# tylerrleee/mcmc-gpu

Measured on AMD Instinct MI355X. Metric: chain-steps/sec on 256x256 grid x 1024 chains; accept-rate parity, higher is better.
Workload: dtype f64; 1 GPU; largeScaleChain 256x256 grid, 1024 chains/GPU, fp64, Philox spectral (Matern 0.9125) proposals, blocks 50-80, sigma_mc 5 (BASELINE configs[1]); chains_total=1024, mh_steps_per_bench_step=2048

## Files before the change

mcmc_gpu_amd/csrc/chain_strip_kernel.hip:

```cpp
#include "gsm_internal.h"
#include "device_util.h"
#include "proposal_device.h"
#include "strip_step.h"
#include <math.h>
#include <stdlib.h>
#include <algorithm>
#include <type_traits>

namespace gsm {

using namespace dev;
using strip::kST;
using strip::kSW;
using strip::kNR;

constexpr int kSUPW = 32 / kSW;
constexpr int kSMAXT = 16 / kSW;

static int strip_tile_len(const BlockTable& B) { return (B.max_bh + 2) * (B.max_bw + 2); }
static int strip_main_len(const FusedArgs& a) { return std::max(a.P.lds_main, strip_tile_len(a.T.B)); }
constexpr int kStripAux = 16 + 32 + 16 + kMathTabDoubles + 4 * kT1S + kMask1D;
size_t fused_strip_lds_doubles(const FusedArgs& a) { return (size_t)strip_main_len(a) + kStripAux; }

bool strip_table_ok(const StaticFields& S, const BlockTable& B, int lds_main, int tiles1_max, int tiles2_max) {
  static int on = -1;
  if (on < 0) { const char* v = getenv("GSM_STRIP"); on = v ? atoi(v) : 1; }
  const size_t lds = ((size_t)std::max(lds_main, strip_tile_len(B)) + kStripAux) * sizeof(double);
  return on && S.sA != nullptr && (uint64_t)S.H * S.W * 48u <= (4ull << 20) && B.n_sizes <= 64 && strip::table_ok(B.max_bh, B.max_bw) &&
         B.max_bh <= kT1S && B.max_bw <= kT1S && (B.masks == nullptr || B.mask1d != nullptr) && lds <= 80 * 1024 && 2 * tiles1_max <= kSW * kSUPW && tiles2_max <= kSW * kSMAXT;
}

using step::crec_t;
using step::load_c;

template <typename TS, bool FAST_DIV, bool NOISE>
__global__ __launch_bounds__(kST, 4) void chain_strip_kernel(const FusedArgs fa) {
  typedef step::cptr_t<FusedArgs> cargs_t;
  auto kargs = [] { return step::kargs<FusedArgs>(); };
  extern __shared__ double lds[];
  double* __restrict__ red = lds + fa.work_len;
  double* __restrict__ red2 = red + 16;
  double* __restrict__ carry = red2 + 32;
  double* __restrict__ mtab = red2 + 32 + 16;
// ... 108 lines not shown
        relaunder();
        nugget_pass<kST, NOISE>(ptid, pa, q, pg, seed, pa.step0 + s, nz, lds, [bw](int y, int x) { return (y + 1) * (bw + 2) + x + 1; }, mtab);
      }
    }
    relaunder();
    const step::Window Gw = step::clip_window(gH, gW, s_row, s_col, s_bh, s_bw);
    strip::Window G;
    {
      const cargs_t K = kargs();
      G = strip::make_window(gH, gW, s_row, s_col, s_bh, s_bw, K->T.S.tr0, K->T.S.tr1, K->T.S.tc0, K->T.S.tc1);
    }
    const strip::Cfg cfg = strip::config(G.wh, G.ww);
    const strip::Lane L = strip::lane_setup(ptid & 63, wave, cfg, G, gH, gW);
    const rsrc_t r_bed = make_rsrc(p_bed, n_cells * (uint32_t)sizeof(TS));
    const rsrc_t r_en = make_rsrc(p_en, n_cells * (uint32_t)sizeof(TS));
    const rsrc_t r_st = make_rsrc(p_st, 3u * n_cells * 16u);
    uint32_t upd_bits;
    double acc_old;
    bool guard;
    {
      double vb[kNR + 2], ve[kNR];
      double2 a2[strip::kNA];
      if (G.interior) strip::load_state<TS, true>(L, cfg.n, gW, r_bed, r_en, r_st, vb, ve, a2);
      else strip::load_state<TS, false>(L, cfg.n, gW, r_bed, r_en, r_st, vb, ve, a2);
      asm volatile("s_waitcnt lgkmcnt(0)\n\ts_barrier" ::: "memory");
      const int ts = s_bw + 2;
      auto field = [&](int jj, bool) { return lds[L.tidx + jj * ts]; };
      if (G.interior) strip::phase_a<TS, true>(L, cfg.n, gW, s_bw, r_st, field, lds, vb, ve, a2, upd_bits, acc_old, guard);
      else strip::phase_a<TS, false>(L, cfg.n, gW, s_bw, r_st, field, lds, vb, ve, a2, upd_bits, acc_old, guard);
    }
    asm volatile("s_waitcnt lgkmcnt(0)\n\ts_barrier" ::: "memory");
    double en[kNR], vn[kNR];
    {
      double acc_new;
      const cargs_t K = kargs();
      const step::StepConsts SC{K->T.S.res, K->T.S.rcp_res, K->T.S.two_res, K->T.S.rcp_two_res};
      if (G.interior) strip::phase_d<TS, FAST_DIV, true>(L, cfg.n, gW, s_bw, r_st, n_cells * 16u, SC, lds, en, acc_new);
      else strip::phase_d<TS, FAST_DIV, false>(L, cfg.n, gW, s_bw, r_st, n_cells * 16u, SC, lds, en, acc_new);
      double delta = acc_new - acc_old;
      if (guard) delta = INFINITY;
      const double w_delta = wave64_sum(delta);
      if (lane == 0) red[wave] = w_delta;
    }
    strip::read_candidate(L, cfg.n, s_bw, lds, vn);
    const double s_hi = carry[0], s_lo = carry[1];
    double loss_prev = carry[2];
    asm volatile("s_waitcnt lgkmcnt(0)\n\ts_barrier" ::: "memory");
    const double sd = strip::waves_sum(red, lane);
    double c_hi, c_lo, loss_next;
    const bool acc = step::decide<FAST_DIV>(sd, sd == INFINITY, s_hi, s_lo, two_sigma2, rcp_two_sigma2, loss_prev, rec->u, c_hi, c_lo, loss_next);
    if (acc) {
      if (G.interior) strip::commit<TS, true, false>(L, cfg.n, gW, r_bed, r_en, r_en, vn, en, upd_bits);
      else strip::commit<TS, false, false>(L, cfg.n, gW, r_bed, r_en, r_en, vn, en, upd_bits);
// ... 23 lines not shown
__global__ __launch_bounds__(kST, 4) void step_strip_kernel(const StepArgs a) {
  extern __shared__ double tile[];
  __shared__ double red[16];
  __shared__ int tab[2 * 64];
  const StaticFields& S = a.S;
  const int tid = threadIdx.x;
  const int lane = tid & 63;
  const int wave = __builtin_amdgcn_readfirstlane(tid >> 6);
  const int chain = blockIdx.x;
  const int H = S.H, W = S.W;
  const uint32_t n_cells = (uint32_t)H * (uint32_t)W;
  const size_t plane = (size_t)H * W;
  const rsrc_t r_bed = make_rsrc((const TS*)a.beds + (size_t)chain * plane, n_cells * (uint32_t)sizeof(TS));
  const rsrc_t r_en = make_rsrc((const TS*)a.energy + (size_t)chain * plane, n_cells * (uint32_t)sizeof(TS));
  const rsrc_t r_rs = make_rsrc(a.resampled + (size_t)chain * plane, n_cells * 4u);
  const rsrc_t r_st = make_rsrc(S.sA, 3u * n_cells * 16u);
  const step::StepConsts SC{S.res, S.rcp_res, S.two_res, S.rcp_two_res};

  double s_hi = a.loss_sum[2 * chain], s_lo = a.loss_sum[2 * chain + 1];
  double loss_prev = (s_hi + s_lo) / S.two_sigma2;
  for (int i = tid; i < a.B.n_sizes; i += kST) { tab[2 * i] = a.B.bh[i]; tab[2 * i + 1] = a.B.bw[i]; }
  if (tid < 16) red[tid] = 0.0;
  const int64_t rin0 = (int64_t)chain * a.in_stride;
  step::ReplayRec nxt = step::read_replay(a, rin0);
  __syncthreads();

  for (int s = 0; s < a.n_steps; ++s) {
    const int64_t rin = rin0 + s;
    const int64_t rout = step::record_index(a, chain, s);
    const step::ReplayRec cur = nxt;
    const bool has_next = s + 1 < a.n_steps;
// ... 4 lines not shown
    }
    const int bh = tab[2 * cur.si], bw = tab[2 * cur.si + 1];
    const rsrc_t r_f = make_rsrc(a.fields + rin * a.field_stride, (uint32_t)(bh * bw) * 8u);
    strip::Window G;
    {
      const step::cptr_t<StepArgs> K = step::kargs<StepArgs>();
      G = strip::uniform(strip::make_window(H, W, cur.row, cur.col, bh, bw, K->S.tr0, K->S.tr1, K->S.tc0, K->S.tc1));
    }
    const strip::Cfg cfg = strip::config(G.wh, G.ww);
    const strip::Lane L = strip::lane_setup(lane, wave, cfg, G, H, W);
    uint32_t upd_bits;
    double acc_old;
    bool guard;
    {
      double vb[kNR + 2], ve[kNR];
      double2 a2[strip::kNA];
      auto field = [&](int jj, bool in) { return ld_f64<2>(r_f, in ? (uint32_t)(L.fidx + jj * bw) * 8u : kOOB); };
      if (G.interior) {
        strip::load_state<TS, true>(L, cfg.n, W, r_bed, r_en, r_st, vb, ve, a2);
        strip::phase_a<TS, true>(L, cfg.n, W, bw, r_st, field, tile, vb, ve, a2, upd_bits, acc_old, guard);
      } else {
        strip::load_state<TS, false>(L, cfg.n, W, r_bed, r_en, r_st, vb, ve, a2);
        strip::phase_a<TS, false>(L, cfg.n, W, bw, r_st, field, tile, vb, ve, a2, upd_bits, acc_old, guard);
      }
    }
    asm volatile("s_waitcnt lgkmcnt(0)\n\ts_barrier" ::: "memory");
    double en[kNR], vn[kNR];
    {
      double acc_new;
      if (G.interior) strip::phase_d<TS, FAST_DIV, true>(L, cfg.n, W, bw, r_st, n_cells * 16u, SC, tile, en, acc_new);
      else strip::phase_d<TS, FAST_DIV, false>(L, cfg.n, W, bw, r_st, n_cells * 16u, SC, tile, en, acc_new);
      double delta = acc_new - acc_old;
      if (guard) delta = INFINITY;
      const double w_delta = wave64_sum(delta);
      if (lane == 0) red[wave] = w_delta;
    }
    strip::read_candidate(L, cfg.n, bw, tile, vn);
    asm volatile("s_waitcnt lgkmcnt(0)\n\ts_barrier" ::: "memory");
    const double sd = strip::waves_sum(red, lane);
    double c_hi, c_lo, loss_next;
    const bool acc = step::decide<FAST_DIV>(sd, sd == INFINITY, s_hi, s_lo, S.two_sigma2, S.rcp_two_sigma2, loss_prev, cur.u, c_hi, c_lo, loss_next);
    if (acc) {
      if (G.interior) strip::commit<TS, true, true>(L, cfg.n, W, r_bed, r_en, r_rs, vn, en, upd_bits);
      else strip::commit<TS, false, true>(L, cfg.n, W, r_bed, r_en, r_rs, vn, en, upd_bits);
      two_sum(c_hi, c_lo, s_hi, s_lo);
      loss_prev = loss_next;
// ... 50 lines not shown
```

mcmc_gpu_amd/csrc/device_util.h:

```cpp
#pragma once
#include <hip/hip_runtime.h>
#include <stdint.h>

namespace gsm {
namespace dev {


constexpr int kNT = 1024;
constexpr int kNW = kNT / 64;
constexpr uint32_t kOOB = 0x80000000u;
constexpr uint64_t kNoUpdBits = 0x7FF8DEADBEEF0001ull;

typedef int v2i32 __attribute__((ext_vector_type(2)));
typedef int v4i32 __attribute__((ext_vector_type(4)));
typedef __amdgpu_buffer_rsrc_t rsrc_t;

__device__ __forceinline__ rsrc_t make_rsrc(const void* p, uint32_t bytes) {
  return __builtin_amdgcn_make_buffer_rsrc(const_cast<void*>(p), 0, (int)bytes, 0x00020000);
}
template <int AUX>
__device__ __forceinline__ double ld_f64(rsrc_t r, uint32_t off) {
  return __builtin_bit_cast(double, __builtin_amdgcn_raw_buffer_load_b64(r, (int)off, 0, AUX));
}
template <int AUX>
__device__ __forceinline__ float ld_f32(rsrc_t r, uint32_t off) {
  return __builtin_bit_cast(float, __builtin_amdgcn_raw_buffer_load_b32(r, (int)off, 0, AUX));
// ... 74 lines not shown
```

mcmc_gpu_amd/csrc/gsm_api.hip:

```cpp
#include "gsm_context.h"
#include "math_tables.h"
#include "normal_score.h"
#include <math.h>
#include <string.h>
#include <algorithm>

using namespace gsm;

static thread_local std::string g_create_err;

int gsm::fail(gsm_handle h, int code, const std::string& msg) {
  if (h) h->err = msg; else g_create_err = msg;
  return code;
}

extern "C" const char* gsm_last_error(gsm_handle h) { return h ? h->err.c_str() : g_create_err.c_str(); }

extern "C" int gsm_create(gsm_handle* out, int32_t H, int32_t W, int32_t n_chains, int32_t dtype, int32_t device) {
  if (!out) return fail(nullptr, GSM_E_ARG, "gsm_create: out is NULL");
  *out = nullptr;
  if (H < 1 || W < 1 || n_chains < 1) return fail(nullptr, GSM_E_ARG, "gsm_create: need H,W >= 1 and n_chains >= 1");
  if ((int64_t)H * W > (1LL << 30)) return fail(nullptr, GSM_E_ARG, "gsm_create: grid too large");
  if (dtype != 0 && dtype != 1) return fail(nullptr, GSM_E_UNSUPPORTED, "gsm_create: dtype must be 0 (fp64 state) or 1 (fp32 state)");
  int ndev = 0;
// ... 64 lines not shown
  S.rcp_two_res = 1.0 / S.two_res;
  S.two_sigma2 = 2 * (sigma_mc * sigma_mc);
  S.rcp_two_sigma2 = 1.0 / S.two_sigma2;
  {
    auto divisor_ok = [](double d) {
      uint64_t bits;
      memcpy(&bits, &d, sizeof(bits));
      const bool all_ones = (bits & 0xFFFFFFFFFFFFFull) == 0xFFFFFFFFFFFFFull;
      return !all_ones && d > 1e-100 && d < 1e100;
    };
    S.fast_div = (divisor_ok(S.res) && divisor_ok(S.two_sigma2)) ? 1 : 0;
  }
  HIPCHK(h, h->d_svx.ensure(n));
  HIPCHK(h, h->d_svy.ensure(n));
  HIPCHK(h, h->d_ds.ensure(n));
  HIPCHK(h, h->d_sABC.ensure(3 * n));
  double2 *sA = h->d_sABC.get(), *sB = sA + n, *sC = sA + 2 * n;
  HIPCHK(h, launch_pack_static(S, h->d_svx.get(), h->d_svy.get(), h->d_ds.get(), st));
  HIPCHK(h, launch_pack_flux_static(S, sA, sB, sC, st));
  S.svx = h->d_svx.get(); S.svy = h->d_svy.get(); S.ds = h->d_ds.get();
  S.sA = sA; S.sB = sB; S.sC = sC;
  HIPCHK(h, hipStreamSynchronize(st));
  h->have_static = true;
  return GSM_OK;
}

extern "C" int gsm_set_blocks(gsm_handle h, int32_t n_sizes, const int32_t* bh, const int32_t* bw,
                              const double* edge_masks_packed, const int64_t* mask_offsets, void* stream) {
  GSM_GRID_HANDLE(h);
  if (n_sizes < 1 || !bh || !bw) return fail(h, GSM_E_ARG, "gsm_set_blocks: empty block table");
  if (n_sizes > 64) return fail(h, GSM_E_UNSUPPORTED, "gsm_set_blocks: at most 64 block sizes");
  hipStream_t st = (hipStream_t)stream;
  HIPCHK(h, hipSetDevice(h->device));
  int max_bh = 0, max_bw = 0, cap = 0;
  int64_t mask_total = 0;
  for (int i = 0; i < n_sizes; ++i) {
// ... 350 lines not shown
```

mcmc_gpu_amd/csrc/gsm_internal.h:

```cpp
#pragma once
#include <hip/hip_runtime.h>
#include <stdint.h>
#include <string>
#include <vector>
#include "../../include/gsm.h"

namespace gsm {

constexpr int kMaxDevices = 64;
inline bool attr_needed_on_this_device(bool (&flags)[kMaxDevices], int& dev) {
  dev = 0;
  if (hipGetDevice(&dev) != hipSuccess || dev < 0 || dev >= kMaxDevices) { dev = -1; return true; }
  return !flags[dev];
}
template <auto K0, auto K1, class... Args>
inline hipError_t launch_pair(bool first, int lds_cap, dim3 grid, dim3 block, size_t lds, hipStream_t st, const Args&... args) {
  static bool attr_set[kMaxDevices] = {};
  int attr_dev;
  if (attr_needed_on_this_device(attr_set, attr_dev)) {
    hipError_t e = hipFuncSetAttribute((const void*)K0, hipFuncAttributeMaxDynamicSharedMemorySize, lds_cap);
    if (e == hipSuccess) e = hipFuncSetAttribute((const void*)K1, hipFuncAttributeMaxDynamicSharedMemorySize, lds_cap);
    if (e != hipSuccess) return e;
    if (attr_dev >= 0) attr_set[attr_dev] = true;
  }
// ... 5 lines not shown
struct StaticFields {
  const double* surf;
  const double* velx;
  const double* vely;
  const double* dhdt;
  const double* smb;
  const double* weight;
  const uint8_t* upd;
  const uint8_t* mc;
  const double2* svx;
  const double2* svy;
  const double2* ds;
  const double2* sA;
  const double2* sB;
  const double2* sC;
  int H, W;
  int32_t tr0, tr1, tc0, tc1;
  double res;
  double two_res;
  double rcp_res;
  double rcp_two_res;
  int fast_div;
  double two_sigma2;
  double rcp_two_sigma2;
};

struct BlockTable {
  const int32_t* bh;
  const int32_t* bw;
  const double* masks;
// ... 285 lines not shown
                     double* out, int64_t n, int inverse, hipStream_t st);
hipError_t launch_qt_groups(const double* quantiles, const double* references, int nq, double clip_min, double clip_max, const double* x,
                            double* out, int n_chains, int plane, const int32_t* group, int inverse, hipStream_t st);
hipError_t launch_sgs_commit_map(int H, int W, int n_chains, double* cur, const double* proposed, uint32_t* resampled, const int32_t* win,
                                 const uint8_t* accept, hipStream_t st);
hipError_t launch_sgs_commit(int H, int W, int n_chains, double* cur, double* next, uint32_t* resampled, const int32_t* win,
                             const uint8_t* accept, hipStream_t st);

hipError_t launch_propose_cholesky(const ProposeArgs& a, const CholArgs& c, hipStream_t st);
hipError_t launch_cholesky_upper(double* A, int n, int ld, double jitter, int* d_info, hipStream_t st);
hipError_t launch_cov_assemble(int bh, int bw, double res, const gsm_vario& v, const double* lag_table, double* sigma,
                               int ld, hipStream_t st);
hipError_t launch_step(const StepArgs& a, hipStream_t st);
hipError_t launch_step_flux(const StepArgs& a, hipStream_t st);
bool step_flux_supported(const StepArgs& a);
hipError_t launch_pack_flux_static(const StaticFields& S, double2* sA, double2* sB, double2* sC, hipStream_t st);
hipError_t launch_init_loss(const StaticFields& S, int n_chains, const void* beds, void* energy, int f32_state,
                            double* loss_sum, double* loss0, hipStream_t st);
hipError_t launch_pack_static(const StaticFields& S, double2* svx, double2* svy, double2* ds, hipStream_t st);
hipError_t launch_residual(const StaticFields& S, int n_chains, const double* beds, double* out, hipStream_t st);
hipError_t launch_propose(const ProposeArgs& a, hipStream_t st);
hipError_t launch_propose_scalars(const ProposeArgs& a, hipStream_t st);
hipError_t launch_debug_normals(uint64_t seed, int64_t step, uint32_t stream_id, uint32_t idx0, int n, const double* mathtab, double* out,
                                hipStream_t st);
hipError_t launch_debug_proposal_math(int which, int model, double smoothness, int64_t n, const void* x0, const double* x1, const double* x2,
                                      const double* x3, const double* mathtab, void* out, hipStream_t st);
hipError_t launch_k2_tables(const BlockTable& B, const int32_t* k2_off, double resolution, double* k2tab, hipStream_t st);
hipError_t launch_spectral_from_noise(const ProposeArgs& a, const int32_t* size_idx, const double* rf_scalars, const double* noise_re,
                                      const double* noise_im, const double* nugget_field, hipStream_t st);
hipError_t launch_chain_fused(const FusedArgs& a, hipStream_t st);
hipError_t launch_chain_strip(const FusedArgs& a, hipStream_t st);
// ... 28 lines not shown
```

mcmc_gpu_amd/csrc/step_flux_kernel.hip:

```cpp
#include "gsm_internal.h"
#include "device_util.h"
#include "step_common.h"
#include <math.h>
#include <stdlib.h>
#include <algorithm>

namespace gsm {

using namespace dev;

size_t step_flux_lds_bytes(int tile_cap) { return ((size_t)2 * tile_cap + 4 * kNW + 64) * sizeof(double); }

template <typename TS, int KT, bool FAST_DIV>
__global__ __launch_bounds__(kNT, 4) void step_flux_kernel(const StepArgs a) {
  constexpr bool F32 = sizeof(TS) == 4;
  extern __shared__ double lds[];
  double* __restrict__ qx = lds;
  double* __restrict__ qy = lds + a.tile_cap;
  double* __restrict__ red = lds + 2 * a.tile_cap;
  int* tab = (int*)(red + 4 * kNW);

  const StaticFields& S = a.S;
  const int tid = threadIdx.x;
  const int lane = tid & 63;
// ... 168 lines not shown
         (uint64_t)a.S.H * a.S.W * 16u < 0x80000000ull;
}

hipError_t launch_step_flux(const StepArgs& a, hipStream_t st) {
  if (!step_flux_supported(a)) return hipErrorInvalidValue;
  if (a.f32_state) {
    if (a.tile_cap <= 2 * kNT) return launch_flux_t<float, 2>(a, st);
    if (a.tile_cap <= 4 * kNT) return launch_flux_t<float, 4>(a, st);
    return launch_flux_t<float, 7>(a, st);
  }
  if (a.tile_cap <= 2 * kNT) return launch_flux_t<double, 2>(a, st);
  if (a.tile_cap <= 4 * kNT) return launch_flux_t<double, 4>(a, st);
  return launch_flux_t<double, 7>(a, st);
}

__global__ __launch_bounds__(256) void pack_flux_static_kernel(const StaticFields S, double2* sA, double2* sB, double2* sC) {
  const int n = S.H * S.W;
  for (int g = blockIdx.x * 256 + threadIdx.x; g < n; g += gridDim.x * 256) {
    const double w = S.weight ? S.weight[g] : 1.0;
    sA[g] = make_double2(S.upd[g] ? w : __builtin_bit_cast(double, kNoUpdBits), S.surf[g]);
    sB[g] = make_double2(S.velx[g], S.vely[g]);
    sC[g] = make_double2(S.mc[g] == 1 ? S.dhdt[g] : __builtin_nan(""), S.smb[g]);
  }
}

hipError_t launch_pack_flux_static(const StaticFields& S, double2* sA, double2* sB, double2* sC, hipStream_t st) {
  int grid = (S.H * S.W + 255) / 256;
  if (grid > 2048) grid = 2048;
  hipLaunchKernelGGL(pack_flux_static_kernel, dim3(grid), dim3(256), 0, st, S, sA, sB, sC);
  return hipGetLastError();
}

}
```

mcmc_gpu_amd/csrc/strip_step.h:

```cpp
#pragma once
#include "gsm_internal.h"
#include "device_util.h"
#include "step_common.h"
#include <math.h>

namespace gsm {
namespace strip {

using namespace dev;

constexpr int kST = 512;
constexpr int kSW = kST / 64;
constexpr int kNR = 16;

struct Cfg { int cs, g, sr, n; };

__host__ __device__ inline int rows_per_strip(int wh, int sr) {
  switch (sr) {
    case 8: return (wh + 7) >> 3;
    case 6: return (int)(((uint32_t)(wh + 5) * 10923u) >> 16);
    case 5: return (int)(((uint32_t)(wh + 4) * 13108u) >> 16);
    case 4: return (wh + 3) >> 2;
    case 2: return (wh + 1) >> 1;
    default: return wh;
// ... 52 lines not shown

enum : uint32_t {
  kFValid = 1u,
  kFColIn = 2u,
  kFColOwn = 4u,
  kFTopIn = 8u,
  kFBelowIn = 16u,
  kFAtLeft = 32u, kFAtRight = 64u,
};
struct Lane {
  uint32_t cell0;
  int fidx;
  int tidx;
  int rows;
  uint32_t flags;
  int lo, hi;
  int jtop, jbot;
};
__host__ __device__ __forceinline__ Lane lane_setup(const int lane, const int wave, const Cfg& c, const Window& g, const int H, const int W) {
  Lane L;
  const int C = 1 << c.cs;
  const int sub = lane >> c.cs, l = lane & (C - 1);
  const int sidx = wave * (64 >> c.cs) + sub;
  const int kr = small_div(sidx, c.g), kc = sidx - kr * c.g;
  const int wc = kc * (C - 2) + l - 1;
  const int gc = g.c0 + wc;
  int rows = min(c.n, g.wh - kr * c.n);
  const bool valid = (kr < c.sr) && (rows > 0) && (wc <= g.ww) && (gc >= 0) && (gc < W);
  if (!valid) rows = -2;
  const bool colin = valid && (wc >= 0) && (wc < g.ww);
  const bool colown = colin && (l >= 1) && (l <= C - 2);
  const int wr0 = kr * c.n - 1;
  const int gr0 = g.r0 + wr0;
  L.rows = rows;
  L.flags = (valid ? kFValid : 0u) | (colin ? kFColIn : 0u) | (colown ? kFColOwn : 0u) | ((valid && kr > 0) ? kFTopIn : 0u) |
            ((valid && kr * c.n + rows < g.wh) ? kFBelowIn : 0u) | ((gc == 0) ? kFAtLeft : 0u) | ((gc == W - 1) ? kFAtRight : 0u);
  L.lo = max(0, -gr0);
  L.hi = valid ? min(rows + 1, H - 1 - gr0) : -1;
  L.jtop = -gr0; L.jbot = H - 1 - gr0;
  L.cell0 = (uint32_t)(gr0 * W + gc);
  L.fidx = (g.mr0 + wr0) * g.bw + g.mc0 + wc;
  L.tidx = (g.mr0 + wr0 + 1) * (g.bw + 2) + g.mc0 + wc + 1;
  return L;
}
__host__ __device__ __forceinline__ bool has(const Lane& L, const uint32_t f) { return (L.flags & f) != 0u; }

__device__ __forceinline__ Lane fresh(Lane L) {
  asm volatile("" : "+v"(L.rows), "+v"(L.flags), "+v"(L.lo), "+v"(L.hi));
  return L;
}
__device__ __forceinline__ int fresh_s(int W) { asm volatile("" : "+s"(W)); return W; }

template <typename TS> struct RowIO;
template <> struct RowIO<double> {
  static __device__ __forceinline__ double load(rsrc_t r, uint32_t off, uint32_t soff) {
    return __builtin_bit_cast(double, __builtin_amdgcn_raw_buffer_load_b64(r, (int)off, (int)soff, 2));
  }
  static __device__ __forceinline__ void store(rsrc_t r, uint32_t off, uint32_t soff, double v) {
    __builtin_amdgcn_raw_buffer_store_b64(__builtin_bit_cast(v2i32, v), r, (int)off, (int)soff, 2);
  }
};
template <> struct RowIO<float> {
  static __device__ __forceinline__ double load(rsrc_t r, uint32_t off, uint32_t soff) {
    return (double)__builtin_bit_cast(float, __builtin_amdgcn_raw_buffer_load_b32(r, (int)off, (int)soff, 2));
  }
  static __device__ __forceinline__ void store(rsrc_t r, uint32_t off, uint32_t soff, double v) {
    __builtin_amdgcn_raw_buffer_store_b32(__builtin_bit_cast(int, (float)v), r, (int)off, (int)soff, 2);
  }
};
__device__ __forceinline__ double ld_f64_s(rsrc_t r, uint32_t off, uint32_t soff) {
  return __builtin_bit_cast(double, __builtin_amdgcn_raw_buffer_load_b64(r, (int)off, (int)soff, 0));
}

template <bool INTERIOR>
__device__ __forceinline__ void row_offsets(const Lane& L, const int jj, const int W, const uint32_t cb, uint32_t& off, uint32_t& soff) {
  if (INTERIOR) { off = L.cell0 * cb; soff = (uint32_t)(jj * W) * cb; }
  else { off = (L.cell0 + (uint32_t)(jj * W)) * cb; soff = 0u; }
}
__host__ __device__ __forceinline__ bool row_exists(const Lane& L, const int jj) { return jj >= L.lo && jj <= L.hi; }
__host__ __device__ __forceinline__ bool row_own(const Lane& L, const int jj) { return (jj >= 1) && (jj <= kNR) && (jj <= L.rows); }
struct WriteMasks { bool w0, w1, w2; };
__host__ __device__ __forceinline__ WriteMasks write_masks(const Lane& L) {
  WriteMasks m;
  const bool valid = has(L, kFValid), colin = has(L, kFColIn);
  m.w0 = valid && !(has(L, kFTopIn) && colin);
  m.w1 = valid && (has(L, kFColOwn) || !colin);
  m.w2 = valid && !(has(L, kFBelowIn) && colin);
  return m;
}
template <bool INTERIOR>
__host__ __device__ __forceinline__ bool cell_written(const Lane& L, const WriteMasks& m, const int jj) {
  bool w = (jj == 0) ? m.w0 : ((jj <= L.rows && m.w1) || (jj - 1 == L.rows && m.w2));
  if (!INTERIOR) w = w && row_exists(L, jj);
  return w;
}

constexpr int kNA = 4;
template <typename TS, bool INTERIOR, int PARTS = 3>
__device__ __forceinline__ void load_state(const Lane& L_in, const int n, const int W_in, const rsrc_t r_bed, const rsrc_t r_en, const rsrc_t r_st,
                                           double (&vb)[kNR + 2], double (&ve)[kNR], double2 (&a2)[kNA]) {
  const Lane L = fresh(L_in);
  const int W = fresh_s(W_in);
  const WriteMasks wm = write_masks(L);
  const bool colown = has(L, kFColOwn);
  uint32_t oob = kOOB;
  asm volatile("" : "+v"(oob));
  const uint32_t ownS = colown ? L.cell0 * (uint32_t)sizeof(TS) : oob, own16 = colown ? L.cell0 * 16u : oob;
#pragma unroll
  for (int jj = 0; jj < kNR + 2; ++jj) {
    if (PARTS & 1) vb[jj] = 0.0;
    if ((PARTS & 2) && jj >= 1 && jj <= kNR) ve[jj - 1] = 0.0;
    if ((PARTS & 2) && jj >= 1 && jj <= kNA) a2[jj - 1] = make_double2(0.0, 0.0);
    if (jj <= n + 1) {
      uint32_t off, soff, off16, soff16;
      row_offsets<INTERIOR>(L, jj, W, (uint32_t)sizeof(TS), off, soff);
      row_offsets<INTERIOR>(L, jj, W, 16u, off16, soff16);
      if (PARTS & 1) vb[jj] = RowIO<TS>::load(r_bed, cell_written<INTERIOR>(L, wm, jj) ? off : oob, soff);
      if ((PARTS & 2) && jj >= 1 && jj <= kNR) {
        const bool ro = row_own(L, jj);
        if (jj <= kNA) a2[jj - 1] = ld_f64x2(r_st, ro ? (INTERIOR ? own16 : (colown ? off16 : oob)) : oob, soff16);
        ve[jj - 1] = RowIO<TS>::load(r_en, ro ? (INTERIOR ? ownS : (colown ? off : oob)) : oob, soff);
      }
    }
  }
}

template <typename TS, bool INTERIOR, class Field>
__device__ __forceinline__ void phase_a(const Lane& L_in, const int n, const int W_in, const int bw, const rsrc_t r_st, Field field,
                                        double* __restrict__ tile, double (&vb)[kNR + 2], double (&ve)[kNR], double2 (&a2)[kNA],
                                        uint32_t& upd_bits, double& acc_old, bool& guard) {
  constexpr bool F32 = sizeof(TS) == 4;
  const Lane L = fresh(L_in);
  const int W = fresh_s(W_in);
  const WriteMasks wm = write_masks(L);
  const bool colown = has(L, kFColOwn);
  uint32_t oob = kOOB;
  asm volatile("" : "+v"(oob));
  const uint32_t own16 = colown ? L.cell0 * 16u : oob;
  guard = false;
  upd_bits = 0u;
  const int ts = bw + 2;
#pragma unroll
  for (int jj = 0; jj < kNR + 2; ++jj) {
    if (jj <= n + 1) {
      double v = vb[jj];
      if (jj >= 1 && jj <= kNR) {
        const bool own = row_own(L, jj) && colown;
        const double2 A2 = a2[(jj - 1) % kNA];
        if (jj + kNA <= kNR && jj + kNA <= n) {
          uint32_t off, soff;
          row_offsets<INTERIOR>(L, jj + kNA, W, 16u, off, soff);
          a2[(jj - 1) % kNA] = ld_f64x2(r_st, row_own(L, jj + kNA) ? (INTERIOR ? own16 : (colown ? off : oob)) : oob, soff);
        }
        const step::Candidate cb = step::candidate_bed<F32>(own, v, field(jj, own), A2);
        v = cb.v;
        guard = guard || cb.grounded;
        upd_bits |= cb.upd ? (1u << jj) : 0u;
      }
      if (cell_written<INTERIOR>(L, wm, jj)) tile[L.tidx + jj * ts] = v;
    }
  }
  __builtin_amdgcn_sched_barrier(0);
  acc_old = 0.0;
#pragma unroll
  for (int R = 1; R <= kNR; ++R) if (R <= n) acc_old += ve[R - 1];
}

template <int CTRL>
__device__ __forceinline__ double wave_shift(double x) {
  const v2i32 b = __builtin_bit_cast(v2i32, x);
  v2i32 o;
  o.x = __builtin_amdgcn_update_dpp(0, b.x, CTRL, 0xF, 0xF, true);
  o.y = __builtin_amdgcn_update_dpp(0, b.y, CTRL, 0xF, 0xF, true);
  return __builtin_bit_cast(double, o);
}
constexpr int kWaveShr1 = 0x138;
constexpr int kWaveShl1 = 0x130;

using step::StepConsts;

struct RowOps { double v, surf; double2 B2, C2; };
template <typename TS, bool FAST_DIV, bool INTERIOR>
struct PhaseD {
  const Lane& L; const int n, W, ts; const rsrc_t r_st; const uint32_t off_sB; const StepConsts& K; const double* __restrict__ tile;
  const uint32_t off_v, off_o;
  const bool colown;
  double (&en)[kNR]; double acc_new;
  double qy_m2, qy_m1, qx_m1; double2 C_m1; bool own_m1;

  __device__ __forceinline__ RowOps request(const int jj) const {
    RowOps o;
    uint32_t ov, oo, soff;
    if (INTERIOR) { ov = off_v; oo = off_o; soff = (uint32_t)(jj * W) * 16u; }
    else {
      const uint32_t off = (L.cell0 + (uint32_t)(jj * W)) * 16u;
      const bool need = row_exists(L, jj);
      ov = need ? off : kOOB; oo = (need && colown) ? off : kOOB; soff = 0u;
    }
    o.v = tile[L.tidx + jj * ts];
    o.surf = ld_f64_s(r_st, ov + 8u, soff);
    o.B2 = ld_f64x2(r_st, ov, soff + off_sB);
    o.C2 = make_double2(0.0, 0.0);
    if (jj >= 1 && jj <= kNR) o.C2 = ld_f64x2(r_st, oo, soff + 2u * off_sB);
    return o;
  }
  template <int JJ>
  __device__ __forceinline__ void row(const RowOps cur) {
    constexpr bool F32 = sizeof(TS) == 4;
    if (JJ <= n + 1) {
      RowOps nxt;
      if constexpr (JJ + 1 <= kNR + 1) nxt = request(JJ + 1);
      const double thick = cur.surf - cur.v;
      const double qx = cur.B2.x * thick, qy = cur.B2.y * thick;
      if (JJ >= 2) {
        constexpr int R = (JJ >= 2) ? JJ - 1 : 1;
        double qxl = wave_shift<kWaveShr1>(qx_m1), qxr = wave_shift<kWaveShl1>(qx_m1);
        double qya = qy_m2, qyb = qy;
        bool xedge = false, yedge = false;
        if (!INTERIOR) {
          const bool atleft = has(L, kFAtLeft), atright = has(L, kFAtRight);
          const bool attop = (R == L.jtop), atbot = (R == L.jbot);
          xedge = atleft || atright; yedge = attop || atbot;
          if (atleft) qxl = qx_m1;
          if (atright) qxr = qx_m1;
          if (attop) qya = qy_m1;
          if (atbot) qyb = qy_m1;
        }
        const double e = step::flux_energy<FAST_DIV, F32, INTERIOR>(qxr - qxl, qyb - qya, !xedge, !yedge, C_m1, K, own_m1);
        en[R - 1] = e;
        acc_new += e;
      }
      qy_m2 = qy_m1; qy_m1 = qy; qx_m1 = qx; C_m1 = cur.C2; own_m1 = row_own(L, JJ) && colown;
      __builtin_amdgcn_sched_barrier(0);
      if constexpr (JJ + 1 <= kNR + 1) row<JJ + 1>(nxt);
    }
  }
};

template <typename TS, bool FAST_DIV, bool INTERIOR>
__device__ __forceinline__ void phase_d(const Lane& L_in, const int n, const int W_in, const int bw, const rsrc_t r_st, const uint32_t off_sB,
                                        const StepConsts& K, const double* __restrict__ tile, double (&en)[kNR], double& acc_new) {
  const Lane L = fresh(L_in);
  const int W = fresh_s(W_in);
#pragma unroll
  for (int R = 0; R < kNR; ++R) en[R] = 0.0;
  const bool colown = has(L, kFColOwn);
  PhaseD<TS, FAST_DIV, INTERIOR> P{L, n, W, bw + 2, r_st, off_sB, K, tile,
                                   has(L, kFValid) ? L.cell0 * 16u : kOOB, colown ? L.cell0 * 16u : kOOB, colown,
                                   en, 0.0, 0.0, 0.0, 0.0, make_double2(0.0, 0.0), false};
  P.template row<0>(P.request(0));
  acc_new = P.acc_new;
}

__device__ __forceinline__ void read_candidate(const Lane& L, const int n, const int bw, const double* __restrict__ tile, double (&vn)[kNR]) {
  const int ts = bw + 2;
#pragma unroll
  for (int R = 1; R <= kNR; ++R) {
    vn[R - 1] = 0.0;
    if (R <= n) vn[R - 1] = tile[L.tidx + R * ts];
  }
}

template <typename TS, bool INTERIOR, bool RS>
__device__ __forceinline__ void commit(const Lane& L_in, const int n, const int W_in, const rsrc_t r_bed, const rsrc_t r_en, const rsrc_t r_rs,
                                       const double (&vn)[kNR], const double (&en)[kNR], const uint32_t upd_bits) {
  const Lane L = fresh(L_in);
// ... 26 lines not shown
```

Baseline: 17.86 million chain-steps/s.

## Split packed static planes into separate weight and surface planes to halve loads

```diff
diff --git a/mcmc_gpu_amd/csrc/chain_strip_kernel.hip b/mcmc_gpu_amd/csrc/chain_strip_kernel.hip
--- a/mcmc_gpu_amd/csrc/chain_strip_kernel.hip
+++ b/mcmc_gpu_amd/csrc/chain_strip_kernel.hip
@@ -26,7 +26,7 @@
   static int on = -1;
   if (on < 0) { const char* v = getenv("GSM_STRIP"); on = v ? atoi(v) : 1; }
   const size_t lds = ((size_t)std::max(lds_main, strip_tile_len(B)) + kStripAux) * sizeof(double);
-  return on && S.sA != nullptr && (uint64_t)S.H * S.W * 48u <= (4ull << 20) && B.n_sizes <= 64 && strip::table_ok(B.max_bh, B.max_bw) &&
+  return on && S.sA != nullptr && S.sS != nullptr && (uint64_t)S.H * S.W * 48u <= (4ull << 20) && B.n_sizes <= 64 && strip::table_ok(B.max_bh, B.max_bw) &&
          B.max_bh <= kT1S && B.max_bw <= kT1S && (B.masks == nullptr || B.mask1d != nullptr) && lds <= 80 * 1024 && 2 * tiles1_max <= kSW * kSUPW && tiles2_max <= kSW * kSMAXT;
 }
 
@@ -165,20 +165,20 @@
     const strip::Lane L = strip::lane_setup(ptid & 63, wave, cfg, G, gH, gW);
     const rsrc_t r_bed = make_rsrc(p_bed, n_cells * (uint32_t)sizeof(TS));
     const rsrc_t r_en = make_rsrc(p_en, n_cells * (uint32_t)sizeof(TS));
-    const rsrc_t r_st = make_rsrc(p_st, 3u * n_cells * 16u);
+    const rsrc_t r_st = make_rsrc(p_st, pack::planes_bytes(n_cells));
     uint32_t upd_bits;
     double acc_old;
     bool guard;
     {
       double vb[kNR + 2], ve[kNR];
-      double2 a2[strip::kNA];
-      if (G.interior) strip::load_state<TS, true>(L, cfg.n, gW, r_bed, r_en, r_st, vb, ve, a2);
-      else strip::load_state<TS, false>(L, cfg.n, gW, r_bed, r_en, r_st, vb, ve, a2);
+      double aw[strip::kNA];
+      if (G.interior) strip::load_state<TS, true>(L, cfg.n, gW, r_bed, r_en, r_st, n_cells * 16u, vb, ve, aw);
+      else strip::load_state<TS, false>(L, cfg.n, gW, r_bed, r_en, r_st, n_cells * 16u, vb, ve, aw);
       asm volatile("s_waitcnt lgkmcnt(0)\n\ts_barrier" ::: "memory");
       const int ts = s_bw + 2;
       auto field = [&](int jj, bool) { return lds[L.tidx + jj * ts]; };
-      if (G.interior) strip::phase_a<TS, true>(L, cfg.n, gW, s_bw, r_st, field, lds, vb, ve, a2, upd_bits, acc_old, guard);
-      else strip::phase_a<TS, false>(L, cfg.n, gW, s_bw, r_st, field, lds, vb, ve, a2, upd_bits, acc_old, guard);
+      if (G.interior) strip::phase_a<TS, true>(L, cfg.n, gW, s_bw, r_st, n_cells * 16u, field, lds, vb, ve, aw, upd_bits, acc_old);
+      else strip::phase_a<TS, false>(L, cfg.n, gW, s_bw, r_st, n_cells * 16u, field, lds, vb, ve, aw, upd_bits, acc_old);
     }
     asm volatile("s_waitcnt lgkmcnt(0)\n\ts_barrier" ::: "memory");
     double en[kNR], vn[kNR];
@@ -186,8 +186,8 @@
       double acc_new;
       const cargs_t K = kargs();
       const step::StepConsts SC{K->T.S.res, K->T.S.rcp_res, K->T.S.two_res, K->T.S.rcp_two_res};
-      if (G.interior) strip::phase_d<TS, FAST_DIV, true>(L, cfg.n, gW, s_bw, r_st, n_cells * 16u, SC, lds, en, acc_new);
-      else strip::phase_d<TS, FAST_DIV, false>(L, cfg.n, gW, s_bw, r_st, n_cells * 16u, SC, lds, en, acc_new);
+      if (G.interior) strip::phase_d<TS, FAST_DIV, true>(L, cfg.n, gW, s_bw, r_st, n_cells * 16u, SC, lds, upd_bits, en, acc_new, guard);
+      else strip::phase_d<TS, FAST_DIV, false>(L, cfg.n, gW, s_bw, r_st, n_cells * 16u, SC, lds, upd_bits, en, acc_new, guard);
       double delta = acc_new - acc_old;
       if (guard) delta = INFINITY;
       const double w_delta = wave64_sum(delta);
@@ -241,7 +241,7 @@
   const rsrc_t r_bed = make_rsrc((const TS*)a.beds + (size_t)chain * plane, n_cells * (uint32_t)sizeof(TS));
   const rsrc_t r_en = make_rsrc((const TS*)a.energy + (size_t)chain * plane, n_cells * (uint32_t)sizeof(TS));
   const rsrc_t r_rs = make_rsrc(a.resampled + (size_t)chain * plane, n_cells * 4u);
-  const rsrc_t r_st = make_rsrc(S.sA, 3u * n_cells * 16u);
+  const rsrc_t r_st = make_rsrc(S.sA, pack::planes_bytes(n_cells));
   const step::StepConsts SC{S.res, S.rcp_res, S.two_res, S.rcp_two_res};
 
   double s_hi = a.loss_sum[2 * chain], s_lo = a.loss_sum[2 * chain + 1];
@@ -276,22 +276,22 @@
     bool guard;
     {
       double vb[kNR + 2], ve[kNR];
-      double2 a2[strip::kNA];
+      double aw[strip::kNA];
       auto field = [&](int jj, bool in) { return ld_f64<2>(r_f, in ? (uint32_t)(L.fidx + jj * bw) * 8u : kOOB); };
       if (G.interior) {
-        strip::load_state<TS, true>(L, cfg.n, W, r_bed, r_en, r_st, vb, ve, a2);
-        strip::phase_a<TS, true>(L, cfg.n, W, bw, r_st, field, tile, vb, ve, a2, upd_bits, acc_old, guard);
+        strip::load_state<TS, true>(L, cfg.n, W, r_bed, r_en, r_st, n_cells * 16u, vb, ve, aw);
+        strip::phase_a<TS, true>(L, cfg.n, W, bw, r_st, n_cells * 16u, field, tile, vb, ve, aw, upd_bits, acc_old);
       } else {
-        strip::load_state<TS, false>(L, cfg.n, W, r_bed, r_en, r_st, vb, ve, a2);
-        strip::phase_a<TS, false>(L, cfg.n, W, bw, r_st, field, tile, vb, ve, a2, upd_bits, acc_old, guard);
+        strip::load_state<TS, false>(L, cfg.n, W, r_bed, r_en, r_st, n_cells * 16u, vb, ve, aw);
+        strip::phase_a<TS, false>(L, cfg.n, W, bw, r_st, n_cells * 16u, field, tile, vb, ve, aw, upd_bits, acc_old);
       }
     }
     asm volatile("s_waitcnt lgkmcnt(0)\n\ts_barrier" ::: "memory");
     double en[kNR], vn[kNR];
     {
       double acc_new;
-      if (G.interior) strip::phase_d<TS, FAST_DIV, true>(L, cfg.n, W, bw, r_st, n_cells * 16u, SC, tile, en, acc_new);
-      else strip::phase_d<TS, FAST_DIV, false>(L, cfg.n, W, bw, r_st, n_cells * 16u, SC, tile, en, acc_new);
+      if (G.interior) strip::phase_d<TS, FAST_DIV, true>(L, cfg.n, W, bw, r_st, n_cells * 16u, SC, tile, upd_bits, en, acc_new, guard);
+      else strip::phase_d<TS, FAST_DIV, false>(L, cfg.n, W, bw, r_st, n_cells * 16u, SC, tile, upd_bits, en, acc_new, guard);
       double delta = acc_new - acc_old;
       if (guard) delta = INFINITY;
       const double w_delta = wave64_sum(delta);
diff --git a/mcmc_gpu_amd/csrc/device_util.h b/mcmc_gpu_amd/csrc/device_util.h
--- a/mcmc_gpu_amd/csrc/device_util.h
+++ b/mcmc_gpu_amd/csrc/device_util.h
@@ -1,6 +1,7 @@
 #pragma once
 #include <hip/hip_runtime.h>
 #include <stdint.h>
+#include "static_pack.h"
 
 namespace gsm {
 namespace dev {
@@ -9,7 +10,7 @@
 constexpr int kNT = 1024;
 constexpr int kNW = kNT / 64;
 constexpr uint32_t kOOB = 0x80000000u;
-constexpr uint64_t kNoUpdBits = 0x7FF8DEADBEEF0001ull;
+using pack::kNoUpdBits;
 
 typedef int v2i32 __attribute__((ext_vector_type(2)));
 typedef int v4i32 __attribute__((ext_vector_type(4)));
diff --git a/mcmc_gpu_amd/csrc/gsm_api.hip b/mcmc_gpu_amd/csrc/gsm_api.hip
--- a/mcmc_gpu_amd/csrc/gsm_api.hip
+++ b/mcmc_gpu_amd/csrc/gsm_api.hip
@@ -102,12 +102,15 @@
   HIPCHK(h, h->d_svx.ensure(n));
   HIPCHK(h, h->d_svy.ensure(n));
   HIPCHK(h, h->d_ds.ensure(n));
-  HIPCHK(h, h->d_sABC.ensure(3 * n));
+  const size_t sabc_bytes = pack::alloc_bytes(n, (size_t)h->W);
+  HIPCHK(h, h->d_sABC.ensure((sabc_bytes + sizeof(double2) - 1) / sizeof(double2)));
   double2 *sA = h->d_sABC.get(), *sB = sA + n, *sC = sA + 2 * n;
+  double *sW = (double*)(sA + 3 * n), *sS = sW + n;
+  HIPCHK(h, hipMemsetAsync(sS + n, 0, sabc_bytes - pack::planes_bytes((uint32_t)n), st));
   HIPCHK(h, launch_pack_static(S, h->d_svx.get(), h->d_svy.get(), h->d_ds.get(), st));
-  HIPCHK(h, launch_pack_flux_static(S, sA, sB, sC, st));
+  HIPCHK(h, launch_pack_flux_static(S, sA, sB, sC, sW, sS, st));
   S.svx = h->d_svx.get(); S.svy = h->d_svy.get(); S.ds = h->d_ds.get();
-  S.sA = sA; S.sB = sB; S.sC = sC;
+  S.sA = sA; S.sB = sB; S.sC = sC; S.sW = sW; S.sS = sS;
   HIPCHK(h, hipStreamSynchronize(st));
   h->have_static = true;
   return GSM_OK;
diff --git a/mcmc_gpu_amd/csrc/gsm_internal.h b/mcmc_gpu_amd/csrc/gsm_internal.h
--- a/mcmc_gpu_amd/csrc/gsm_internal.h
+++ b/mcmc_gpu_amd/csrc/gsm_internal.h
@@ -4,6 +4,7 @@
 #include <string>
 #include <vector>
 #include "../../include/gsm.h"
+#include "static_pack.h"
 
 namespace gsm {
 
@@ -43,6 +44,8 @@
   const double2* sA;
   const double2* sB;
   const double2* sC;
+  const double* sW;
+  const double* sS;
   int H, W;
   int32_t tr0, tr1, tc0, tc1;
   double res;
@@ -358,7 +361,7 @@
 hipError_t launch_step(const StepArgs& a, hipStream_t st);
 hipError_t launch_step_flux(const StepArgs& a, hipStream_t st);
 bool step_flux_supported(const StepArgs& a);
-hipError_t launch_pack_flux_static(const StaticFields& S, double2* sA, double2* sB, double2* sC, hipStream_t st);
+hipError_t launch_pack_flux_static(const StaticFields& S, double2* sA, double2* sB, double2* sC, double* sW, double* sS, hipStream_t st);
 hipError_t launch_init_loss(const StaticFields& S, int n_chains, const void* beds, void* energy, int f32_state,
                             double* loss_sum, double* loss0, hipStream_t st);
 hipError_t launch_pack_static(const StaticFields& S, double2* svx, double2* svy, double2* ds, hipStream_t st);
diff --git a/mcmc_gpu_amd/csrc/static_pack.h b/mcmc_gpu_amd/csrc/static_pack.h
--- /dev/null
+++ b/mcmc_gpu_amd/csrc/static_pack.h
@@ -0,0 +1,36 @@
+#pragma once
+#include <stdint.h>
+#include <string.h>
+
+#if defined(__HIPCC__)
+#define GSM_PACK_HD __host__ __device__
+#else
+#define GSM_PACK_HD
+#endif
+
+namespace gsm {
+namespace pack {
+
+constexpr uint64_t kNoUpdBits = 0x7FF8DEADBEEF0001ull;
+constexpr int kTailRows = 18;
+
+GSM_PACK_HD inline uint32_t off_sB(uint32_t n) { return 16u * n; }
+GSM_PACK_HD inline uint32_t off_sC(uint32_t n) { return 32u * n; }
+GSM_PACK_HD inline uint32_t off_sW(uint32_t n) { return 48u * n; }
+GSM_PACK_HD inline uint32_t off_sS(uint32_t n) { return 56u * n; }
+GSM_PACK_HD inline uint32_t planes_bytes(uint32_t n) { return 64u * n; }
+inline size_t alloc_bytes(size_t n, size_t W) { return 64u * n + (size_t)kTailRows * W * 8u; }
+
+GSM_PACK_HD inline uint64_t wupd_bits(bool upd, double w) {
+  uint64_t b;
+  memcpy(&b, &w, sizeof(b));
+  return upd ? b : kNoUpdBits;
+}
+GSM_PACK_HD inline uint64_t f64_bits(double v) {
+  uint64_t b;
+  memcpy(&b, &v, sizeof(b));
+  return b;
+}
+
+}
+}
diff --git a/mcmc_gpu_amd/csrc/step_flux_kernel.hip b/mcmc_gpu_amd/csrc/step_flux_kernel.hip
--- a/mcmc_gpu_amd/csrc/step_flux_kernel.hip
+++ b/mcmc_gpu_amd/csrc/step_flux_kernel.hip
@@ -206,20 +206,23 @@
   return launch_flux_t<double, 7>(a, st);
 }
 
-__global__ __launch_bounds__(256) void pack_flux_static_kernel(const StaticFields S, double2* sA, double2* sB, double2* sC) {
+__global__ __launch_bounds__(256) void pack_flux_static_kernel(const StaticFields S, double2* sA, double2* sB, double2* sC, uint64_t* sW, uint64_t* sS) {
   const int n = S.H * S.W;
   for (int g = blockIdx.x * 256 + threadIdx.x; g < n; g += gridDim.x * 256) {
     const double w = S.weight ? S.weight[g] : 1.0;
-    sA[g] = make_double2(S.upd[g] ? w : __builtin_bit_cast(double, kNoUpdBits), S.surf[g]);
+    const uint64_t wb = pack::wupd_bits(S.upd[g] != 0, w), sb = pack::f64_bits(S.surf[g]);
+    sA[g] = make_double2(__builtin_bit_cast(double, wb), __builtin_bit_cast(double, sb));
     sB[g] = make_double2(S.velx[g], S.vely[g]);
     sC[g] = make_double2(S.mc[g] == 1 ? S.dhdt[g] : __builtin_nan(""), S.smb[g]);
-  }
-}
-
-hipError_t launch_pack_flux_static(const StaticFields& S, double2* sA, double2* sB, double2* sC, hipStream_t st) {
+    sW[g] = wb;
+    sS[g] = sb;
+  }
+}
+
+hipError_t launch_pack_flux_static(const StaticFields& S, double2* sA, double2* sB, double2* sC, double* sW, double* sS, hipStream_t st) {
   int grid = (S.H * S.W + 255) / 256;
   if (grid > 2048) grid = 2048;
-  hipLaunchKernelGGL(pack_flux_static_kernel, dim3(grid), dim3(256), 0, st, S, sA, sB, sC);
+  hipLaunchKernelGGL(pack_flux_static_kernel, dim3(grid), dim3(256), 0, st, S, sA, sB, sC, (uint64_t*)sW, (uint64_t*)sS);
   return hipGetLastError();
 }
 
diff --git a/mcmc_gpu_amd/csrc/strip_step.h b/mcmc_gpu_amd/csrc/strip_step.h
--- a/mcmc_gpu_amd/csrc/strip_step.h
+++ b/mcmc_gpu_amd/csrc/strip_step.h
@@ -90,8 +90,7 @@
   int tidx;
   int rows;
   uint32_t flags;
-  int lo, hi;
-  int jtop, jbot;
+  int hi, jtop;
 };
 __host__ __device__ __forceinline__ Lane lane_setup(const int lane, const int wave, const Cfg& c, const Window& g, const int H, const int W) {
   Lane L;
@@ -111,9 +110,8 @@
   L.rows = rows;
   L.flags = (valid ? kFValid : 0u) | (colin ? kFColIn : 0u) | (colown ? kFColOwn : 0u) | ((valid && kr > 0) ? kFTopIn : 0u) |
             ((valid && kr * c.n + rows < g.wh) ? kFBelowIn : 0u) | ((gc == 0) ? kFAtLeft : 0u) | ((gc == W - 1) ? kFAtRight : 0u);
-  L.lo = max(0, -gr0);
   L.hi = valid ? min(rows + 1, H - 1 - gr0) : -1;
-  L.jtop = -gr0; L.jbot = H - 1 - gr0;
+  L.jtop = -gr0;
   L.cell0 = (uint32_t)(gr0 * W + gc);
   L.fidx = (g.mr0 + wr0) * g.bw + g.mc0 + wc;
   L.tidx = (g.mr0 + wr0 + 1) * (g.bw + 2) + g.mc0 + wc + 1;
@@ -122,7 +120,7 @@
 __host__ __device__ __forceinline__ bool has(const Lane& L, const uint32_t f) { return (L.flags & f) != 0u; }
 
 __device__ __forceinline__ Lane fresh(Lane L) {
-  asm volatile("" : "+v"(L.rows), "+v"(L.flags), "+v"(L.lo), "+v"(L.hi));
+  asm volatile("" : "+v"(L.rows), "+v"(L.flags), "+v"(L.jtop), "+v"(L.hi));
   return L;
 }
 __device__ __forceinline__ int fresh_s(int W) { asm volatile("" : "+s"(W)); return W; }
@@ -147,13 +145,19 @@
 __device__ __forceinline__ double ld_f64_s(rsrc_t r, uint32_t off, uint32_t soff) {
   return __builtin_bit_cast(double, __builtin_amdgcn_raw_buffer_load_b64(r, (int)off, (int)soff, 0));
 }
+static_assert(pack::kTailRows == kNR + 2, "static_pack.h: the tail behind sS holds the rows phase D reads past the grid");
+__device__ __forceinline__ uint32_t plane_sW(const uint32_t off_sB) { return 3u * off_sB; }
+__device__ __forceinline__ uint32_t plane_sS(const uint32_t off_sB) { return 3u * off_sB + (off_sB >> 1); }
+__device__ __forceinline__ double ld_wupd(rsrc_t r, uint32_t off, uint32_t soff, const uint32_t off_sB) {
+  return ld_f64_s(r, off, soff + plane_sW(off_sB));
+}
 
 template <bool INTERIOR>
 __device__ __forceinline__ void row_offsets(const Lane& L, const int jj, const int W, const uint32_t cb, uint32_t& off, uint32_t& soff) {
   if (INTERIOR) { off = L.cell0 * cb; soff = (uint32_t)(jj * W) * cb; }
   else { off = (L.cell0 + (uint32_t)(jj * W)) * cb; soff = 0u; }
 }
-__host__ __device__ __forceinline__ bool row_exists(const Lane& L, const int jj) { return jj >= L.lo && jj <= L.hi; }
+__host__ __device__ __forceinline__ bool row_exists(const Lane& L, const int jj) { return jj >= L.jtop && jj <= L.hi; }
 __host__ __device__ __forceinline__ bool row_own(const Lane& L, const int jj) { return (jj >= 1) && (jj <= kNR) && (jj <= L.rows); }
 struct WriteMasks { bool w0, w1, w2; };
 __host__ __device__ __forceinline__ WriteMasks write_masks(const Lane& L) {
@@ -173,28 +177,29 @@
 
 constexpr int kNA = 4;
 template <typename TS, bool INTERIOR, int PARTS = 3>
-__device__ __forceinline__ void load_state(const Lane& L_in, const int n, const int W_in, const rsrc_t r_bed, const rsrc_t r_en, const rsrc_t r_st,
-                                           double (&vb)[kNR + 2], double (&ve)[kNR], double2 (&a2)[kNA]) {
+__device__ __forceinline__ void load_state(const Lane& L_in, const int n, const int W_in, const rsrc_t r_bed, const rsrc_t r_en, const rsrc_t r_st, const uint32_t off_sB_in,
+                                           double (&vb)[kNR + 2], double (&ve)[kNR], double (&aw)[kNA]) {
   const Lane L = fresh(L_in);
   const int W = fresh_s(W_in);
+  const uint32_t off_sB = (uint32_t)fresh_s((int)off_sB_in);
   const WriteMasks wm = write_masks(L);
   const bool colown = has(L, kFColOwn);
   uint32_t oob = kOOB;
   asm volatile("" : "+v"(oob));
-  const uint32_t ownS = colown ? L.cell0 * (uint32_t)sizeof(TS) : oob, own16 = colown ? L.cell0 * 16u : oob;
+  const uint32_t ownS = colown ? L.cell0 * (uint32_t)sizeof(TS) : oob, own8 = colown ? L.cell0 * 8u : oob;
 #pragma unroll
   for (int jj = 0; jj < kNR + 2; ++jj) {
     if (PARTS & 1) vb[jj] = 0.0;
     if ((PARTS & 2) && jj >= 1 && jj <= kNR) ve[jj - 1] = 0.0;
-    if ((PARTS & 2) && jj >= 1 && jj <= kNA) a2[jj - 1] = make_double2(0.0, 0.0);
+    if ((PARTS & 2) && jj >= 1 && jj <= kNA) aw[jj - 1] = 0.0;
     if (jj <= n + 1) {
-      uint32_t off, soff, off16, soff16;
+      uint32_t off, soff, off8, soff8;
       row_offsets<INTERIOR>(L, jj, W, (uint32_t)sizeof(TS), off, soff);
-      row_offsets<INTERIOR>(L, jj, W, 16u, off16, soff16);
+      row_offsets<INTERIOR>(L, jj, W, 8u, off8, soff8);
       if (PARTS & 1) vb[jj] = RowIO<TS>::load(r_bed, cell_written<INTERIOR>(L, wm, jj) ? off : oob, soff);
       if ((PARTS & 2) && jj >= 1 && jj <= kNR) {
         const bool ro = row_own(L, jj);
-        if (jj <= kNA) a2[jj - 1] = ld_f64x2(r_st, ro ? (INTERIOR ? own16 : (colown ? off16 : oob)) : oob, soff16);
+        if (jj <= kNA) aw[jj - 1] = ld_wupd(r_st, ro ? (INTERIOR ? own8 : (colown ? off8 : oob)) : oob, soff8, off_sB);
         ve[jj - 1] = RowIO<TS>::load(r_en, ro ? (INTERIOR ? ownS : (colown ? off : oob)) : oob, soff);
       }
     }
@@ -202,19 +207,20 @@
 }
 
 template <typename TS, bool INTERIOR, class Field>
-__device__ __forceinline__ void phase_a(const Lane& L_in, const int n, const int W_in, const int bw, const rsrc_t r_st, Field field,
-                                        double* __restrict__ tile, double (&vb)[kNR + 2], double (&ve)[kNR], double2 (&a2)[kNA],
-                                        uint32_t& upd_bits, double& acc_old, bool& guard) {
+__device__ __forceinline__ void phase_a(const Lane& L_in, const int n, const int W_in, const int bw, const rsrc_t r_st, const uint32_t off_sB_in, Field field,
+                                        double* __restrict__ tile, double (&vb)[kNR + 2], double (&ve)[kNR], double (&aw)[kNA],
+                                        uint32_t& upd_bits, double& acc_old) {
   constexpr bool F32 = sizeof(TS) == 4;
   const Lane L = fresh(L_in);
   const int W = fresh_s(W_in);
+  const uint32_t off_sB = (uint32_t)fresh_s((int)off_sB_in);
   const WriteMasks wm = write_masks(L);
   const bool colown = has(L, kFColOwn);
   uint32_t oob = kOOB;
   asm volatile("" : "+v"(oob));
-  const uint32_t own16 = colown ? L.cell0 * 16u : oob;
-  guard = false;
+  const uint32_t own8 = colown ? L.cell0 * 8u : oob;
   upd_bits = 0u;
+  acc_old = 0.0;
   const int ts = bw + 2;
 #pragma unroll
   for (int jj = 0; jj < kNR + 2; ++jj) {
@@ -222,24 +228,20 @@
       double v = vb[jj];
       if (jj >= 1 && jj <= kNR) {
         const bool own = row_own(L, jj) && colown;
-        const double2 A2 = a2[(jj - 1) % kNA];
+        const double wupd = aw[(jj - 1) % kNA];
         if (jj + kNA <= kNR && jj + kNA <= n) {
           uint32_t off, soff;
-          row_offsets<INTERIOR>(L, jj + kNA, W, 16u, off, soff);
-          a2[(jj - 1) % kNA] = ld_f64x2(r_st, row_own(L, jj + kNA) ? (INTERIOR ? own16 : (colown ? off : oob)) : oob, soff);
+          row_offsets<INTERIOR>(L, jj + kNA, W, 8u, off, soff);
+          aw[(jj - 1) % kNA] = ld_wupd(r_st, row_own(L, jj + kNA) ? (INTERIOR ? own8 : (colown ? off : oob)) : oob, soff, off_sB);
         }
-        const step::Candidate cb = step::candidate_bed<F32>(own, v, field(jj, own), A2);
+        const step::Candidate cb = step::candidate_bed<F32>(own, v, field(jj, own), make_double2(wupd, 0.0));
         v = cb.v;
-        guard = guard || cb.grounded;
         upd_bits |= cb.upd ? (1u << jj) : 0u;
       }
       if (cell_written<INTERIOR>(L, wm, jj)) tile[L.tidx + jj * ts] = v;
-    }
-  }
-  __builtin_amdgcn_sched_barrier(0);
-  acc_old = 0.0;
-#pragma unroll
-  for (int R = 1; R <= kNR; ++R) if (R <= n) acc_old += ve[R - 1];
+      if (jj >= 1 && jj <= kNR && jj <= n) acc_old += ve[jj - 1];
+    }
+  }
 }
 
 template <int CTRL>
@@ -262,6 +264,7 @@
   const uint32_t off_v, off_o;
   const bool colown;
   double (&en)[kNR]; double acc_new;
+  const uint32_t upd_bits; bool guard;
   double qy_m2, qy_m1, qx_m1; double2 C_m1; bool own_m1;
 
   __device__ __forceinline__ RowOps request(const int jj) const {
@@ -274,7 +277,7 @@
       ov = need ? off : kOOB; oo = (need && colown) ? off : kOOB; soff = 0u;
     }
     o.v = tile[L.tidx + jj * ts];
-    o.surf = ld_f64_s(r_st, ov + 8u, soff);
+    o.surf = ld_f64_s(r_st, ov >> 1, (soff >> 1) + plane_sS(off_sB));
     o.B2 = ld_f64x2(r_st, ov, soff + off_sB);
     o.C2 = make_double2(0.0, 0.0);
     if (jj >= 1 && jj <= kNR) o.C2 = ld_f64x2(r_st, oo, soff + 2u * off_sB);
@@ -287,6 +290,7 @@
       RowOps nxt;
       if constexpr (JJ + 1 <= kNR + 1) nxt = request(JJ + 1);
       const double thick = cur.surf - cur.v;
+      if (JJ >= 1 && JJ <= kNR) guard = guard || (((upd_bits >> JJ) & 1u) != 0u && thick <= 0.0);
       const double qx = cur.B2.x * thick, qy = cur.B2.y * thick;
       if (JJ >= 2) {
         constexpr int R = (JJ >= 2) ? JJ - 1 : 1;
@@ -295,7 +299,7 @@
         bool xedge = false, yedge = false;
         if (!INTERIOR) {
           const bool atleft = has(L, kFAtLeft), atright = has(L, kFAtRight);
-          const bool attop = (R == L.jtop), atbot = (R == L.jbot);
+          const bool attop = (R == L.jtop), atbot = (R == L.hi);
           xedge = atleft || atright; yedge = attop || atbot;
           if (atleft) qxl = qx_m1;
           if (atright) qxr = qx_m1;
@@ -315,7 +319,7 @@
 
 template <typename TS, bool FAST_DIV, bool INTERIOR>
 __device__ __forceinline__ void phase_d(const Lane& L_in, const int n, const int W_in, const int bw, const rsrc_t r_st, const uint32_t off_sB,
-                                        const StepConsts& K, const double* __restrict__ tile, double (&en)[kNR], double& acc_new) {
+                                        const StepConsts& K, const double* __restrict__ tile, const uint32_t upd_bits, double (&en)[kNR], double& acc_new, bool& guard) {
   const Lane L = fresh(L_in);
   const int W = fresh_s(W_in);
 #pragma unroll
@@ -323,9 +327,10 @@
   const bool colown = has(L, kFColOwn);
   PhaseD<TS, FAST_DIV, INTERIOR> P{L, n, W, bw + 2, r_st, off_sB, K, tile,
                                    has(L, kFValid) ? L.cell0 * 16u : kOOB, colown ? L.cell0 * 16u : kOOB, colown,
-                                   en, 0.0, 0.0, 0.0, 0.0, make_double2(0.0, 0.0), false};
+                                   en, 0.0, upd_bits, false, 0.0, 0.0, 0.0, make_double2(0.0, 0.0), false};
   P.template row<0>(P.request(0));
   acc_new = P.acc_new;
+  guard = P.guard;
 }
 
 __device__ __forceinline__ void read_candidate(const Lane& L, const int n, const int bw, const double* __restrict__ tile, double (&vn)[kNR]) {
```

Result: faster. 18.07 million chain-steps/s (median of 6 runs) (+1.2%).
